# computablee/heterogeneous-spmv

Measured on AMD Instinct MI355X. Metric: SpMV GFLOP/s and achieved HBM GB/s (fp64) per matrix, 1/2/4/8 MI355X, higher is better.
Workload: dtype f64

## Files before the change

### heterogeneous-spmv_amd/cli/cli_common.h

```cpp
#pragma once
#include <math.h>
#include <stdio.h>
#include <stdlib.h>
#include <string.h>

#include <chrono>
#include <string>
#include <vector>

#include "hspmv.h"

namespace cli {

struct Options {
  int gpus = 1;
  int dtype = HSPMV_F64;
  bool x_rand = false;
  unsigned long long seed = 42;
  unsigned kernel = HSPMV_KERNEL_AUTO;
  unsigned lanes = 0;
  bool nt = false;
  int plan = HSPMV_CSR3_PLAN_AUTO;
  int deterministic = 0;
  bool check = true;
  std::string dump_y;
  std::string params = "mi355x";
  bool bandk = true;
};

inline bool ends_with(const std::string &s, const char *suf) {
  const size_t n = strlen(suf);
  return s.size() >= n && s.compare(s.size() - n, n, suf) == 0;
}

inline bool parse_options(int argc, char **argv, int first, Options &o) {
  for (int i = first; i < argc; ++i) {
    std::string a = argv[i];
    auto need = [&](const char *name) -> const char * {
// ... 28 lines not shown
      } else { fprintf(stderr, "bad --kernel %s\n", v); return false; }
    } else if (a == "--nt") {
      o.nt = true;
    } else if (a == "--plan") {
      const char *v = need("--plan"); if (!v) return false;
      if (!strcmp(v, "aligned")) o.plan = HSPMV_CSR3_PLAN_ALIGNED;
      else if (!strcmp(v, "packed")) o.plan = HSPMV_CSR3_PLAN_PACKED;
      else if (!strcmp(v, "ssr")) o.plan = HSPMV_CSR3_PLAN_SSR;
      else { fprintf(stderr, "bad --plan %s\n", v); return false; }
    } else if (a == "--deterministic") {
      o.deterministic = HSPMV_DETERMINISTIC_ORDERED;
    } else if (a == "--reproducible") {
      o.deterministic = HSPMV_DETERMINISTIC_REPRODUCIBLE;
    } else if (a == "--serial") {
      o.deterministic = HSPMV_DETERMINISTIC_SERIAL;
    } else if (a == "--no-check") {
      o.check = false;
    } else if (a == "--dump-y") {
      const char *v = need("--dump-y"); if (!v) return false;
      o.dump_y = v;
    } else if (a == "--file-order") {
      o.bandk = false;
    } else if (a == "--params") {
      const char *v = need("--params"); if (!v) return false;
      o.params = v;
    } else {
      fprintf(stderr, "unknown option %s\n", a.c_str());
      return false;
    }
  }
// ... 64 lines not shown
  int ndev = 0;
  if (hspmv_device_count(&ndev) != HSPMV_OK) return die("hspmv_device_count");
  const int gpus = o.gpus > 0 ? o.gpus : ndev;
  std::vector<int> devs((size_t)(gpus > 0 ? gpus : 1));
  for (size_t p = 0; p < devs.size(); ++p) devs[p] = (int)p;
  hspmv_options opt;
  memset(&opt, 0, sizeof(opt));
  opt.struct_size = sizeof(opt);
  opt.flags = flags_of(o);
  opt.devices = gpus > 1 ? devs.data() : nullptr;
  opt.n_devices = gpus > 1 ? gpus : 0;
  opt.csr3_plan = o.plan;
  opt.deterministic = o.deterministic;
  if (hspmv_create_ex(&h, &view, mv.n_ssr > 0 ? &mv : nullptr, &opt) != HSPMV_OK)
    return die("hspmv_create_ex");
  std::vector<double> x64;
  fill_x(o, A.n, x64);
  if (perm) {
    std::vector<double> xf(x64);
    for (int64_t i = 0; i < A.n; ++i) x64[(size_t)i] = xf[(size_t)perm[i]];
  }
  std::vector<float> x32;
  const void *xp = x64.data();
  if (A.dtype == HSPMV_F32) {
    x32.assign(x64.begin(), x64.end());
    xp = x32.data();
  }
  if (hspmv_set_x(h, xp) != HSPMV_OK) return die("hspmv_set_x");
  hspmv_timing t;
  if (hspmv_run(h, 5, num_runs, &t) != HSPMV_OK) return die("hspmv_run");
// ... 66 lines not shown
```

### heterogeneous-spmv_amd/cli/spmv_csr.cpp

```cpp
#include "cli_common.h"

int main(int argc, char **argv) {
  if (argc < 3) {
    printf("%s inputfile.csr num_runs [--gpus N] [--dtype f32|f64] [--x ones|rand:SEED] "
           "[--kernel auto|stream|vector[:L]] [--nt] [--dump-y PATH] [--no-check]\n",
           argv[0]);
    return 0;
  }
  cli::Options o;
  if (!cli::parse_options(argc, argv, 3, o)) return 1;
  const int num_runs = atoi(argv[2]);
  if (num_runs < 1) {
    fprintf(stderr, "num_runs must be >= 1\n");
    return 1;
  }
  printf("Before Read\n");
  hspmv_csr_buf A;
  hspmv_csr3_buf maps;
  if (cli::read_matrix(argv[1], o.dtype, A, maps) != HSPMV_OK) return cli::die("read");
  printf("After Read\n");
  if (A.dtype != o.dtype) {
    fprintf(stderr, "matrix file holds dtype %d, requested %d\n", A.dtype, o.dtype);
    return 1;
  }
// ... 9 lines not shown
```

### heterogeneous-spmv_amd/csrc/hspmv_api.cpp

```cpp
#include <string.h>

#include <algorithm>
#include <chrono>
#include <cstddef>
#include <memory>
#include <vector>

#include "hspmv_runtime.h"

using namespace hspmv;

namespace {

int check_handle(hspmv_handle *h) {
  if (!h || h->shards.empty()) return set_error(HSPMV_E_INVALID, "invalid handle");
  return HSPMV_OK;
}

int create_single(hspmv_handle **hp, const hspmv_csr *A, const hspmv_csr3_maps *maps, int device,
                  void *stream, unsigned flags, const Tuning &tune) {
  ContigScope contig(tune);
  if (int rc0 = check_deterministic(flags, tune)) return rc0;
  const bool devptrs = (flags & HSPMV_FLAG_DEVICE_PTRS) != 0;
  if (!A) return set_error(HSPMV_E_INVALID, "matrix is NULL");
// ... 68 lines not shown
    }
  }
  if ((rc = finish_shard(s, A->dtype, flags, stream))) {
    free_shard(s, h->borrowed);
    return rc;
  }
  if (!devptrs && (rc = place_shard(s, A->n, A->dtype))) {
    free_shard(s, h->borrowed);
    return rc;
  }
  (void)ncclGetVersion(&h->rccl_version);
  *hp = h.release();
  return HSPMV_OK;
}

int check_devices(const int *devices, int n, int *ndev_out) {
  int ndev = 0;
  if (hipGetDeviceCount(&ndev) != hipSuccess || ndev < 1)
    return set_error(HSPMV_E_NODEV, "no HIP device available");
  *ndev_out = ndev;
  for (int p = 0; devices && p < n; ++p)
    if (devices[p] < 0 || devices[p] >= ndev)
      return set_error(HSPMV_E_NODEV, "device %d out of range (have %d)", devices[p], ndev);
  return HSPMV_OK;
}

}

extern "C" {

// ... 130 lines not shown
  if (!h || gpu < 0 || gpu >= (int)h->shards.size()) return nullptr;
  return (void *)h->shards[gpu].x;
}

void *hspmv_y_device(hspmv_handle *h, int gpu) {
  if (!h || gpu < 0 || gpu >= (int)h->shards.size()) return nullptr;
  return h->shards[gpu].y;
}

int hspmv_spmv(hspmv_handle *h) {
  int rc;
  if ((rc = check_handle(h))) return rc;
  if (!h->x_set) return set_error(HSPMV_E_STATE, "x not set (hspmv_set_x / hspmv_bind_x_device)");
  for (auto &s : h->shards) {
    HIP_TRY(hipSetDevice(s.device));
    hipError_t e = launch_spmv(s.A, s.dp, h->dtype, s.plan, s.x, s.y, s.stream);
    if (e != hipSuccess)
      return set_error(HSPMV_E_HIP, "SpMV launch on GPU %d failed: %s", s.device, hipGetErrorString(e));
  }
  return HSPMV_OK;
}

int hspmv_synchronize(hspmv_handle *h) {
  clear_error();
  int rc;
  if ((rc = check_handle(h))) return rc;
  for (auto &s : h->shards) {
    HIP_TRY(hipSetDevice(s.device));
    HIP_TRY(hipStreamSynchronize(s.stream));
  }
  return HSPMV_OK;
}

int hspmv_run(hspmv_handle *h, int warmup, int iters, hspmv_timing *out) {
  clear_error();
  int rc;
  if ((rc = check_handle(h))) return rc;
  if (!out || iters < 1 || warmup < 0) return set_error(HSPMV_E_INVALID, "bad arguments");
  for (int i = 0; i < warmup; ++i) {
    if ((rc = hspmv_spmv(h))) return rc;
    if ((rc = hspmv_synchronize(h))) return rc;
  }
  double tmin = 1e30, tmax = 0, tsum = 0, wmin = 1e30, wmax = 0, wsum = 0;
  for (int i = 0; i < iters; ++i) {
    auto tic = std::chrono::steady_clock::now();
    for (auto &s : h->shards) {
      HIP_TRY(hipSetDevice(s.device));
      HIP_TRY(hipEventRecord(s.ev0, s.stream));
      hipError_t e = launch_spmv(s.A, s.dp, h->dtype, s.plan, s.x, s.y, s.stream);
      if (e != hipSuccess)
        return set_error(HSPMV_E_HIP, "SpMV launch failed: %s", hipGetErrorString(e));
      HIP_TRY(hipEventRecord(s.ev1, s.stream));
    }
    double dev = 0.0;
    for (auto &s : h->shards) {
      HIP_TRY(hipSetDevice(s.device));
      HIP_TRY(hipEventSynchronize(s.ev1));
      float ms = 0.f;
      HIP_TRY(hipEventElapsedTime(&ms, s.ev0, s.ev1));
      dev = std::max(dev, (double)ms * 1e-3);
    }
    const double wall = std::chrono::duration<double>(std::chrono::steady_clock::now() - tic).count();
    tmin = std::min(tmin, dev); tmax = std::max(tmax, dev); tsum += dev;
    wmin = std::min(wmin, wall); wmax = std::max(wmax, wall); wsum += wall;
  }
  memset(out, 0, sizeof(*out));
  out->t_min = tmin; out->t_max = tmax; out->t_avg = tsum / iters;
  out->wall_min = wmin; out->wall_max = wmax; out->wall_avg = wsum / iters;
// ... 92 lines not shown
  out->csr3_plan = s.plan.kernel != kCsr3 ? 0
                   : s.A.n_ssr == 0 ? HSPMV_CSR3_PLAN_ROW_GROUPS
                   : s.tune.csr3_plan == HSPMV_CSR3_PLAN_SSR ? HSPMV_CSR3_PLAN_SSR
                   : csr3_fill(s.tune) ? HSPMV_CSR3_PLAN_ALIGNED : HSPMV_CSR3_PLAN_PACKED;
  out->csort_slot_bytes = s.plan.kernel == kCsort ? (s.dp.cs.slot32 ? 4 : 8) : 0;
  out->csort_row_blocks = s.plan.kernel == kCsort ? s.dp.cs.row_blocks : 0;
  out->rccl_version = h->rccl_version;
  out->slab_kernel_rule = s.heavy_frac < 0 ? 0 : (s.A.slab_stream ? 2 : 1);
  out->heavy_group_frac = s.heavy_frac < 0 ? 0.0 : s.heavy_frac;
  out->lds_pad = s.plan.lds_pad ? 1 : 0;
  out->csort_fixed_point = s.plan.kernel == kCsort && s.dp.cs.fixed ? 1 : 0;
  out->serial_order = 1;
  for (auto &sh : h->shards) out->serial_order &= sh.dp.serial_max == INT32_MAX ? 1 : 0;
  out->row_slices = s.dp.sl_desc ? 1 : 0;
  out->slice_pos_bits = s.dp.sl_desc ? s.dp.sl_pos_bits : 0;
  if (s.plan.kernel == kCsort)
    for (int hh = 0; hh < 4; ++hh) out->csort_part_begin[hh] = s.csort_part_begin[hh];
  for (auto &sh : h->shards)
    if (sh.plan.kernel == kCsort) {
      out->csort_chunks += sh.csort_chunks;
      out->csort_seg_chunks += sh.csort_seg_chunks;
    }
  return HSPMV_OK;
}

extern "C" {

static_assert(sizeof(hspmv_info) >= HSPMV_INFO_SIZE_1_0, "hspmv_info shrank below its 1.0 layout");
static_assert(offsetof(hspmv_info, heavy_group_frac) + sizeof(double) == HSPMV_INFO_SIZE_1_0,
              "HSPMV_INFO_SIZE_1_0 must end at the last 1.0 field");
// ... 55 lines not shown
```

### heterogeneous-spmv_amd/csrc/hspmv_internal.h

```cpp
#pragma once
#include <hip/hip_runtime_api.h>
#include <stdint.h>

#include "hspmv.h"

namespace hspmv {

struct DevCSR {
  int32_t m = 0;
  int64_t n = 0;
  int64_t nnz = 0;
  const int32_t *row_ptr = nullptr;
  const int32_t *col_idx = nullptr;
  const void *val = nullptr;
  int32_t n_ssr = 0, n_sr = 0;
  const int32_t *outer = nullptr;
  const int32_t *inner = nullptr;
  const uint16_t *col16 = nullptr;
  const int32_t *cbase = nullptr;
  const uint64_t *cplanes = nullptr;
  int32_t n_cplanes = 0, cplane_words = 0;
  int32_t c16_mode = 1;
  int32_t col_span_bits = 0;
  bool has_xwin = false, has_xdict = false;
// ... 61 lines not shown

inline int32_t split_threshold(unsigned flags) {
  return (flags & HSPMV_FLAG_NO_SPLIT) ? INT32_MAX : kLongRow;
}

constexpr double kMallResident = 192.0 * 1024 * 1024;
inline double footprint_bytes(int64_t m, int64_t n, int64_t nnz, int dtype) {
  const double sv = dtype == HSPMV_F64 ? 8.0 : 4.0;
  return (double)nnz * (sv + 4.0) + (double)m * (sv + 4.0) + (double)n * sv;
}
inline bool mall_resident(int64_t m, int64_t n, int64_t nnz, int dtype) {
  return footprint_bytes(m, n, nnz, dtype) <= kMallResident;
}
constexpr double kXcdL2Bytes = 4.0 * 1024 * 1024;

inline unsigned flag_kernel(unsigned flags) { return flags & HSPMV_KERNEL_MASK; }
inline int flag_lanes(unsigned flags) { return (int)((flags & HSPMV_LANES_MASK) >> HSPMV_LANES_SHIFT); }
inline int flag_u(unsigned flags) { return (int)((flags >> HSPMV_U_SHIFT) & 0x1Fu); }
inline int32_t flag_xcd_chunk(unsigned flags) {
  const unsigned code = (flags >> HSPMV_XCD_CHUNK_SHIFT) & 0x1Fu;
  return code ? 1 << (code - 1) : 0;
}
inline int32_t flag_groups(unsigned flags) {
  const unsigned code = (flags >> HSPMV_GROUPS_SHIFT) & 0x7u;
  return code ? 1 << (code - 1) : 1;
}

constexpr int kCsortThreads = 1024;
constexpr int kCsortMaxLds = 160 * 1024;
constexpr int kCsortTraceSlots = 4 + 2 * (kCsortThreads / 64);
// ... 59 lines not shown
  const int32_t *slab_col = nullptr;
  const void *slab_val = nullptr;
  DevCsort cs;
};

struct LaunchPlan {
  int kernel = kStream;
  int lanes = 64;
  int waves_per_block = 4;
  int u = 8;
  bool nontemporal = false;
  bool prefetch = false;
  bool y_nt = false;
  int32_t dyn_lds = 0;
  int32_t xcd_chunk = 1;
  int32_t groups = 1;
  int32_t carry = 0;
  bool lds_pad = false;
  bool row_slices = false;
  int64_t blocks = 0;
};

inline int ssr_waves(double rows_per_ssr) {
  const double w = rows_per_ssr / 64.0;
  return w >= 6.0 ? 8 : (w >= 3.0 ? 4 : (w >= 1.5 ? 2 : 1));
}

LaunchPlan plan_launch(const DevCSR &A, int dtype, unsigned flags, double rows_per_ssr,
                       int64_t packed_tasks, const Tuning &t);

hipError_t launch_rows_f32(const DevCSR &A, const DevPlan &dp, const LaunchPlan &p,
                           const float *x, float *y, hipStream_t st);
hipError_t launch_rows_f64(const DevCSR &A, const DevPlan &dp, const LaunchPlan &p,
                           const double *x, double *y, hipStream_t st);

hipError_t launch_csort(const DevCsort &c, int dtype, const void *x, void *y, hipStream_t st);

hipError_t launch_spmv(const DevCSR &A, const DevPlan &dp, int dtype, const LaunchPlan &plan,
                       const void *x, void *y, hipStream_t stream);

}
```

### heterogeneous-spmv_amd/csrc/hspmv_runtime.h

```cpp
#pragma once
#include <hip/hip_runtime_api.h>
#include <rccl/rccl.h>

#include <algorithm>
#include <cstdint>
#include <thread>
#include <vector>

#include "hspmv_common.h"
#include "hspmv_internal.h"

#define HIP_TRY(expr)                                                              \
  do {                                                                             \
    hipError_t _e = (expr);                                                        \
    if (_e != hipSuccess)                                                          \
      return set_error(HSPMV_E_HIP, "%s failed: %s (%s:%d)", #expr,                \
                       hipGetErrorString(_e), __FILE__, __LINE__);                 \
  } while (0)

namespace hspmv {

struct Shard {
  int device = 0;
  hipStream_t stream = nullptr;
// ... 74 lines not shown
  int64_t m = 0, n = 0, nnz = 0;
  int dtype = HSPMV_F64;
  int64_t n_ssr = 0, n_sr = 0;
  unsigned flags = 0;
  bool x_set = false;
  bool borrowed = false;
  int64_t max_rows = 0;
  bool sharded = false;
  int64_t x_entries() const {
    int64_t t = 0;
    for (auto &s : shards) t += s.x_entries;
    return t;
  }
  std::vector<ncclComm_t> comms;
  int rccl_version = 0;
};

namespace hspmv {

template <typename F>
inline void parallel_ranges(int64_t n, int64_t grain, F &&body) {
  const int nt = (int)std::max<int64_t>(1, std::min<int64_t>(16, n / grain));
  if (nt == 1) return (void)body((int64_t)0, n, 0);
  std::vector<std::thread> th;
  for (int t = 0; t < nt; ++t) th.emplace_back([&, t]() { body(n * t / nt, n * (t + 1) / nt, t); });
  for (auto &x : th) x.join();
}

int tuning_from_options(const hspmv_options *o, Tuning *t);
void tuning_from_env(Tuning *t);
// ... 90 lines not shown
```

### heterogeneous-spmv_amd/csrc/spmv_device.cuh

```cuda
#pragma once
#include <hip/hip_runtime.h>

#include "hspmv_internal.h"

namespace hspmv {
namespace dev {

#ifndef HSPMV_DIAG
#define HSPMV_DIAG 0
#endif

constexpr int kTraceWaves = 1 << 17;
constexpr int kTraceSlots = 8;
#if (HSPMV_DIAG & 8)
static __device__ unsigned long long g_trace[kTraceWaves * kTraceSlots];
__device__ __forceinline__ unsigned long long diag_stamp() {
  unsigned long long t;
  asm volatile("s_waitcnt vmcnt(0) lgkmcnt(0)\n\ts_memtime %0\n\ts_waitcnt lgkmcnt(0)"
               : "=s"(t)::"memory");
  return t;
}
#define HSPMV_TRACE(ts, i, v)            \
  do {                                   \
    if ((ts) != nullptr && lane == 0) (ts)[i] = (v); \
// ... 6 lines not shown
#if (HSPMV_DIAG & 512)
#if !(HSPMV_DIAG & 8)
static __device__ unsigned long long g_trace[kTraceWaves * kTraceSlots];
#endif
__device__ __forceinline__ unsigned long long diag_realtime() {
  unsigned long long t;
  asm volatile("s_memrealtime %0\n\ts_waitcnt lgkmcnt(0)" : "=s"(t)::"memory");
  return t;
}
#endif

constexpr int kWave = 64;
#ifndef HSPMV_COOP_GROUPS
#define HSPMV_COOP_GROUPS 1
#endif
constexpr int kNumXcd = 8;

template <bool PAD>
__device__ __forceinline__ int32_t lds_ix(int32_t i) { return PAD ? i + (i >> 5) : i; }
template <int U, bool PAD>
constexpr int wave_lds() {
  return kWave * U + (PAD ? 2 * U : 0);
}

template <bool NT, typename T>
__device__ __forceinline__ T ldg(const T *p) {
  if constexpr (NT)
    return __builtin_nontemporal_load(p);
  else
    return *p;
}
// ... 44 lines not shown
  v += dpp_move<0x118, 0xf>(v);
  return v;
}

template <typename T>
__device__ __forceinline__ T wave_sum_dpp(T v) {
  v += dpp_move<0x111, 0xf>(v);
  v += dpp_move<0x112, 0xf>(v);
  v += dpp_move<0x114, 0xf>(v);
  v += dpp_move<0x118, 0xf>(v);
  v += dpp_move<0x142, 0xa>(v);
  v += dpp_move<0x143, 0xc>(v);
  return lane_value(v, 63);
}

__device__ __forceinline__ uint32_t xcd_chunk_remap(uint32_t b, uint32_t nb, uint32_t s) {
  if (s <= 1) return b;
  const uint32_t span = kNumXcd * s;
  if (b >= (nb / span) * span) return b;
  const uint32_t i = b / kNumXcd, x = b % kNumXcd;
  return (i / s) * span + x * s + (i % s);
}

__device__ __forceinline__ unsigned long long bits_from(int i) {
  return i >= 64 ? 0ull : (~0ull << i);
}

typedef __attribute__((address_space(1))) const char gchar;

template <bool NT, typename T>
__device__ __forceinline__ T ld_off(const gchar *base, uint32_t byte_off) {
  const __attribute__((address_space(1))) T *p =
      (const __attribute__((address_space(1))) T *)(base + byte_off);
  if constexpr (NT)
    return __builtin_nontemporal_load(p);
  else
    return *p;
// ... 298 lines not shown
    }
    T v[kBatch];
#pragma unroll
    for (int j = 0; j < kBatch; ++j)
      v[j] = ld_off<false, T>(xb, (uint32_t)(min(e[j], total - 1) + d[j]) * (uint32_t)sizeof(T));
#pragma unroll
    for (int j = 0; j < kBatch; ++j)
      if (e[j] < total) xs[e[j]] = v[j];
  }
  __syncthreads();
  if constexpr ((HSPMV_DIAG & (64 | 128)) != 0) __builtin_amdgcn_s_setprio(0);
}

template <typename T, bool NT, int U, bool PF, int C16, bool XW, bool XD, int W = 4, bool PAD = false>
__global__ __launch_bounds__(W * 64) void hspmv_csr_stream(
    int32_t m, int32_t long_t, int32_t serial_max, uint32_t xcd_chunk, int32_t groups, int32_t y_nt,
    int32_t carry,
    const int32_t *__restrict__ rp, ColSrc cs, const int2 *__restrict__ xwin, XDict xd,
    const T *__restrict__ val, const T *__restrict__ x, T *__restrict__ y) {
  static_assert(!XD || W == 4, "dictionaries are planned for 256-row blocks");
  __shared__ T lds[W * wave_lds<U, PAD>()];
  __shared__ T xlds[XW ? W * kXWin : 1];
  extern __shared__ __attribute__((aligned(16))) unsigned char xdyn[];
  const int wid = threadIdx.x >> 6;
  const int lane = threadIdx.x & (kWave - 1);
  const int64_t blk = xcd_chunk_remap(blockIdx.x, gridDim.x, xcd_chunk);
  if constexpr (XD) stage_xdict<T, 256>(reinterpret_cast<T *>(xdyn), x, xd, blk, threadIdx.x);
  int64_t g0 = (blk * W + wid) * (int64_t)groups * kWave;
  if (g0 >= m) return;
  const int64_t gend = min<int64_t>(g0 + (int64_t)groups * kWave, m);
  T *my = lds + wid * wave_lds<U, PAD>();
  unsigned long long *ts = nullptr;
#if (HSPMV_DIAG & 8)
  const int64_t wv = blk * W + wid;
  if (wv < kTraceWaves) ts = g_trace + wv * kTraceSlots;
  HSPMV_TRACE(ts, 0, diag_stamp());
  {
    unsigned hw;
    asm volatile("s_getreg_b32 %0, hwreg(HW_REG_HW_ID)" : "=s"(hw));
    HSPMV_TRACE(ts, 6, (unsigned long long)hw);
  }
// ... 18 lines not shown
    int32_t gbase = 0;
    if constexpr (C16 == 2) gbase = (int32_t)sload_i64(cs.cbase, (uint64_t)(g0 / kWave) * 4u);
    wave_rows<T, NT, U, PF, C16, XW, XD, false, PAD>((int32_t)g0, g1, beg, end, long_t, serial_max, cs, val,
                                                     x, y, my,
                                         lane, win, y_nt != 0, carry != 0, gbase, ts);
    ts = nullptr;
    if (g1 >= gend) break;
    g0 = g1;
    beg = nbeg;
    end = nend;
  }
}

template <typename T, bool NT, int U, bool PF, int C16, int W, bool XW, bool XD>
__global__ __launch_bounds__(W * 64) void hspmv_csr3(
    int32_t n_tasks, int32_t long_t, int32_t serial_max, uint32_t xcd_chunk, int32_t y_nt, int32_t carry,
    int32_t align,
    const int32_t *__restrict__ task_start, const int2 *__restrict__ xwin, XDict xd,
    const int32_t *__restrict__ rp, ColSrc cs, const T *__restrict__ val,
    const T *__restrict__ x, T *__restrict__ y) {
  __shared__ T lds[W * wave_lds<U, false>()];
  __shared__ T xlds[XW ? W * kXWin : 1];
  extern __shared__ __attribute__((aligned(16))) unsigned char xdyn[];
  const int wid = threadIdx.x >> 6;
  const int lane = threadIdx.x & (kWave - 1);
  const int64_t blk = xcd_chunk_remap(blockIdx.x, gridDim.x, xcd_chunk);
#if (HSPMV_DIAG & 512)
  unsigned long long *bt = blk < kTraceWaves ? g_trace + blk * kTraceSlots : nullptr;
  if (bt && threadIdx.x == 0) {
    bt[0] = diag_realtime();
    bt[6] = __builtin_amdgcn_s_getreg((31 << 11) | 4);
    bt[7] = __builtin_amdgcn_s_getreg((31 << 11) | 20);
  }
#endif
  if constexpr (XD) stage_xdict<T, W * 64>(reinterpret_cast<T *>(xdyn), x, xd, blk, threadIdx.x);
  const int64_t t = blk * W + wid;
  if (t >= n_tasks) return;
#if (HSPMV_DIAG & 8)
  const unsigned long long tb_stamp = diag_stamp();
#endif
  const int64_t tb = sload_i64(task_start, (uint64_t)t * 4u);
// ... 161 lines not shown
#pragma unroll
  for (int i = 0; i < B; ++i) {
    const int g = i / 4, r = i % 4;
    const uint32_t p = (full || k0 + 4 * g + 4 <= w) ? slice_pos<PB>(q.pq, i) : q.ps[r < 3 ? r : 0];
    xv[i] = xs[p];
  }
#pragma unroll
  for (int i = 0; i < B; ++i) {
    const T p = q.v[i] * xv[i];
    acc = (k0 + i < len) ? acc + p : acc;
  }
  return acc;
}

template <typename T, bool NT, int B, int PB>
__global__ __launch_bounds__(256) void hspmv_slices(int32_t n_slices, uint32_t xcd_chunk, int32_t y_nt,
                                                    Slices sl, XDict xd, const T *__restrict__ val,
                                                    const T *__restrict__ x, T *__restrict__ y) {
  static_assert(B % 4 == 0 && B >= 4, "batches hold whole position groups");
  static_assert(PB == 16 || (PB == 12 && B % 8 == 0), "12-bit positions come in groups of 8 slots");
  extern __shared__ __attribute__((aligned(16))) unsigned char xdyn[];
  const int wid = threadIdx.x >> 6;
  const int lane = threadIdx.x & (kWave - 1);
  const int64_t blk = xcd_chunk_remap(blockIdx.x, gridDim.x, xcd_chunk);
  const int64_t t = blk * 4 + wid;
  int32_t off = 0, poff = 0, w = 0, r0 = 0, nr = 0;
  if (t < n_slices) {
    const sl_i4 d = sload_i128(sl.desc, (uint64_t)t * 8u);
    off = d[0];
    r0 = d[1];
    w = d[2] - d[0];
    nr = d[3] - d[1];
    poff = PB == 12 ? sload_i32(sl.ppre, (uint64_t)t * 4u) : off;
  }
  int32_t len = 0;
  if (lane < nr) len = (int32_t)sl.len[r0 + lane];
  stage_xdict<T, 256>(reinterpret_cast<T *>(xdyn), x, xd, blk, threadIdx.x);
  if (nr <= 0) return;
  const T *xs = reinterpret_cast<const T *>(xdyn);
// ... 25 lines not shown
  if (w > wf) slice_load_tail<T, NT, B, PB>(tail, vb, pb, wf, w, lane);
  __builtin_amdgcn_sched_barrier(0);
  if (wf > 0) acc = slice_consume<T, B, PB>(acc, cur, xs, wf - B, w, len, true);
  if (w > wf) acc = slice_consume<T, B, 16>(acc, tail, xs, wf, w, len, false);
  if constexpr ((HSPMV_DIAG & 256) != 0) {
    if (lane < nr && acc == T(12345.678)) y[r0 + lane] = acc;
  } else if (lane < nr) {
    if (y_nt)
      __builtin_nontemporal_store(acc, y + r0 + lane);
    else
      y[r0 + lane] = acc;
  }
}


template <typename T, int PB>
void launch_slices_pb(const DevPlan &dp, const LaunchPlan &p, const T *x, T *y, hipStream_t st) {
  const Slices sl{dp.sl_desc, dp.sl_len, dp.sl_pos, dp.sl_ppre};
  const XDict xd{dp.xd_blk, reinterpret_cast<const int2 *>(dp.xd_runs)};
  const unsigned dyn = (unsigned)dp.xd_lds_bytes + (unsigned)p.dyn_lds;
  const T *val = static_cast<const T *>(dp.sl_val);
  if (p.nontemporal)
    hipLaunchKernelGGL((hspmv_slices<T, true, HSPMV_SLICE_BATCH, PB>), dim3((unsigned)p.blocks), dim3(256), dyn,
                       st, dp.n_slices, (uint32_t)p.xcd_chunk, (int32_t)p.y_nt, sl, xd, val, x, y);
  else
    hipLaunchKernelGGL((hspmv_slices<T, false, HSPMV_SLICE_BATCH, PB>), dim3((unsigned)p.blocks), dim3(256), dyn,
                       st, dp.n_slices, (uint32_t)p.xcd_chunk, (int32_t)p.y_nt, sl, xd, val, x, y);
}

template <typename T>
hipError_t launch_slices(const DevPlan &dp, const LaunchPlan &p, const T *x, T *y, hipStream_t st) {
  if (!dp.xd_blk || !dp.sl_len || !dp.sl_pos || !dp.sl_val || p.waves_per_block != 4 ||
      p.blocks != ((int64_t)dp.n_slices + 3) / 4 ||
      !(dp.sl_pos_bits == 16 || (dp.sl_pos_bits == 12 && dp.sl_ppre)))
    return hipErrorInvalidValue;
  if (dp.sl_pos_bits == 12)
    launch_slices_pb<T, 12>(dp, p, x, y, st);
  else
    launch_slices_pb<T, 16>(dp, p, x, y, st);
  return hipGetLastError();
}

inline ColSrc col_src(const DevCSR &A) {
  return ColSrc{A.col_idx, A.col16, A.cbase, A.cplanes, A.n_cplanes, A.cplane_words};
}

template <typename T, bool NT, int U, bool PF, int C16, bool XD>
void launch_rows_u(const DevCSR &A, const DevPlan &dp, const LaunchPlan &p, const T *x, T *y,
                   hipStream_t st) {
  const T *val = static_cast<const T *>(A.val);
  const ColSrc cs = col_src(A);
  const XDict xd{dp.xd_blk, reinterpret_cast<const int2 *>(dp.xd_runs)};
  const unsigned dyn = XD ? (unsigned)dp.xd_lds_bytes + (unsigned)p.dyn_lds : (unsigned)p.dyn_lds;
  if (p.kernel == kStream) {
    const int2 *xw = reinterpret_cast<const int2 *>(dp.xwin);
#define HSPMV_STREAM(C, XW, XDX, W, PAD)                                                            \
  hipLaunchKernelGGL((hspmv_csr_stream<T, NT, U, PF, C, XW, XDX, W, PAD>), dim3((unsigned)p.blocks), \
                     dim3(W * 64), dyn, st, A.m, dp.long_t, dp.serial_max, (uint32_t)p.xcd_chunk,       \
                     (int32_t)p.groups,                                                               \
                     (int32_t)p.y_nt, p.carry, A.row_ptr, cs, xw, xd, val, x, y)
    if constexpr (XD) {
      HSPMV_STREAM(false, false, true, 4, false);
      return;
    }
    if constexpr (!PF) {
      if (p.lds_pad) {
        if (p.waves_per_block == 1 && xw) HSPMV_STREAM(C16, true, false, 1, true);
        else if (p.waves_per_block == 1) HSPMV_STREAM(C16, false, false, 1, true);
        else if (p.waves_per_block != 4 && xw) HSPMV_STREAM(C16, true, false, 2, true);
        else if (p.waves_per_block != 4) HSPMV_STREAM(C16, false, false, 2, true);
        else if (xw) HSPMV_STREAM(C16, true, false, 4, true);
        else HSPMV_STREAM(C16, false, false, 4, true);
        return;
// ... 1 lines not shown
    }
    if (p.waves_per_block == 1 && xw) HSPMV_STREAM(C16, true, false, 1, false);
    else if (p.waves_per_block == 1) HSPMV_STREAM(C16, false, false, 1, false);
    else if (p.waves_per_block != 4 && xw) HSPMV_STREAM(C16, true, false, 2, false);
    else if (p.waves_per_block != 4) HSPMV_STREAM(C16, false, false, 2, false);
    else if (xw) HSPMV_STREAM(C16, true, false, 4, false);
    else HSPMV_STREAM(C16, false, false, 4, false);
#undef HSPMV_STREAM
    return;
  }
  {
  const int2 *xw = reinterpret_cast<const int2 *>(dp.xwin);
#define HSPMV_CSR3(W, C, XW, X)                                                               \
  hipLaunchKernelGGL((hspmv_csr3<T, NT, U, PF, C, W, XW, X>), dim3((unsigned)p.blocks),      \
                     dim3(W * 64), dyn, st, dp.n_tasks, dp.long_t, dp.serial_max,             \
                     (uint32_t)p.xcd_chunk,                                                   \
                     (int32_t)p.y_nt, p.carry, dp.task_align, dp.task_start, xw, xd, A.row_ptr, cs, \
                     val, x, y)
  if constexpr (XD) {
    if (p.waves_per_block == 8)
      HSPMV_CSR3(8, false, false, true);
    else
      HSPMV_CSR3(4, false, false, true);
    return;
  } else {
    if (xw && p.waves_per_block == 4) {
      HSPMV_CSR3(4, C16, true, false);
      return;
    }
    switch (p.waves_per_block) {
      case 1: HSPMV_CSR3(1, C16, false, false); break;
// ... 57 lines not shown
```

### heterogeneous-spmv_amd/csrc/spmv_kernels.hip

```cpp
#include <hip/hip_runtime.h>

#include <cstdlib>

#include "hspmv_internal.h"

namespace hspmv {
namespace {

constexpr int kWave = 64;

template <bool NT, typename T>
__device__ __forceinline__ T ldg(const T *p) {
  if constexpr (NT)
    return __builtin_nontemporal_load(p);
  else
    return *p;
}

template <typename T>
__device__ __forceinline__ T wave_sum(T v) {
#pragma unroll
  for (int off = 32; off > 0; off >>= 1) v += __shfl_xor(v, off, kWave);
  return v;
}
// ... 204 lines not shown
                       dp.long_row, rp, ci, val, x, y, static_cast<T *>(nullptr));
    e = hipGetLastError();
  } else if (dp.n_long > 0) {
    hipLaunchKernelGGL((hspmv_long_chunks<T, NT>), dim3((unsigned)dp.n_chunks), dim3(256), 0, st,
                       dp.n_chunks, dp.chunk_k, ci, val, x, static_cast<T *>(dp.partials));
    hipLaunchKernelGGL((hspmv_long_reduce<T>), dim3((unsigned)((dp.n_long + 3) / 4)), dim3(256),
                       0, st, dp.n_long, dp.long_row, dp.long_cstart,
                       static_cast<const T *>(dp.partials), y);
    e = hipGetLastError();
  }
  return e;
}

}

hipError_t launch_spmv(const DevCSR &A, const DevPlan &dp, int dtype, const LaunchPlan &plan,
                       const void *x, void *y, hipStream_t stream) {
  if (dtype == 1) {
    return plan.nontemporal
               ? launch_typed<double, true>(A, dp, plan, (const double *)x, (double *)y, stream)
               : launch_typed<double, false>(A, dp, plan, (const double *)x, (double *)y, stream);
  }
  return plan.nontemporal
             ? launch_typed<float, true>(A, dp, plan, (const float *)x, (float *)y, stream)
             : launch_typed<float, false>(A, dp, plan, (const float *)x, (float *)y, stream);
}

}
```

### heterogeneous-spmv_amd/hspmv/_lib.py

```python
from __future__ import annotations

import ctypes as C
import os
from pathlib import Path

PKG_ROOT = Path(__file__).resolve().parent.parent
REPO_ROOT = PKG_ROOT.parent
LIB_PATH = Path(os.environ.get("HSPMV_LIB", PKG_ROOT / "build" / "libhspmv.so.1"))
HEADER = REPO_ROOT / "include" / "hspmv.h"

F32, F64 = 0, 1

KERNEL_AUTO, KERNEL_VECTOR, KERNEL_STREAM, KERNEL_CSR3, KERNEL_CSORT = 0, 1, 2, 3, 4
LANES_SHIFT = 4
FLAG_NO_COL16 = 1 << 11
FLAG_NONTEMPORAL = 1 << 12
FLAG_DEVICE_PTRS = 1 << 13
FLAG_NO_XCD_REMAP = 1 << 14
FLAG_NO_SPLIT = 1 << 15
U_SHIFT = 16
FLAG_PREFETCH = 1 << 21
FLAG_XCD_REMAP = 1 << 22
FLAG_COL16 = 1 << 23
XCD_CHUNK_SHIFT = 24
# ... 75 lines not shown
                ("n_split_rows", C.c_int32), ("xcd_remap", C.c_int32), ("groups_per_wave", C.c_int32),
                ("x_entries", C.c_int64), ("format_bytes", C.c_double), ("col16", C.c_int32),
                ("wave_tasks", C.c_int32), ("x_windows", C.c_int32), ("x_dict", C.c_int32),
                ("x_dict_entries", C.c_int64), ("x_slabs", C.c_int32),
                ("col16_group", C.c_int32), ("csort_parts", C.c_int32),
                ("placement_trials", C.c_int32), ("placement_pick", C.c_int32),
                ("placement_us", C.c_double * 8),
                ("deterministic", C.c_int32), ("csr3_plan", C.c_int32),
                ("csort_slot_bytes", C.c_int32), ("csort_row_blocks", C.c_int32),
                ("rccl_version", C.c_int32), ("reserved0", C.c_int32),
                ("csort_chunks", C.c_int64), ("csort_seg_chunks", C.c_int64),
                ("slab_kernel_rule", C.c_int32), ("lds_pad", C.c_int32),
                ("heavy_group_frac", C.c_double),
                ("csort_fixed_point", C.c_int32), ("serial_order", C.c_int32),
                ("csort_part_begin", C.c_int64 * 4),
                ("row_slices", C.c_int32), ("slice_pos_bits", C.c_int32)]


CSR3_PLANS = {"auto": 0, "aligned": 1, "packed": 2, "ssr": 3}
DETERMINISTIC = {"any": 0, "ordered": 1, "reproducible": 2, "serial": 3}
SLICES_WHY = {0: "ok", 1: "off", 2: "no_dict", 3: "shape", 4: "chunked", 5: "split_rows",
              6: "long_row", 7: "bytes", 8: "resident"}
CSR3_PLAN_NAMES = {0: None, 1: "aligned", 2: "packed", 3: "ssr", 4: "row_groups"}


class Options(C.Structure):
    _fields_ = [("struct_size", C.c_uint32), ("flags", C.c_uint32),
                ("devices", C.POINTER(C.c_int)), ("n_devices", C.c_int32),
                ("device", C.c_int32), ("stream", C.c_void_p),
                ("csr3_plan", C.c_int32), ("task_nnz", C.c_int32), ("x_windows", C.c_int32),
                ("x_dict", C.c_int32), ("x_dict_cap", C.c_int32), ("x_slabs", C.c_int32),
                ("col16_group", C.c_int32), ("csort", C.c_int32), ("csort_parts", C.c_int32),
                ("csort_chunk_u", C.c_int32), ("stream_waves", C.c_int32),
                ("deterministic", C.c_int32), ("placement_trials", C.c_int32),
                ("row_slices", C.c_int32)]

    TUNABLE = ("csr3_plan", "task_nnz", "x_windows", "x_dict", "x_dict_cap", "x_slabs",
# ... 29 lines not shown
SIGNATURES = {
    "hspmv_create": (C.c_int, [C.POINTER(_H), C.POINTER(Csr), C.POINTER(Csr3Maps), C.c_int, C.c_uint]),
    "hspmv_create_on_device": (C.c_int, [C.POINTER(_H), C.POINTER(Csr), C.POINTER(Csr3Maps),
                                         C.c_int, _P, C.c_uint]),
    "hspmv_create_sharded": (C.c_int, [C.POINTER(_H), C.POINTER(Csr), C.POINTER(Csr3Maps),
                                       C.POINTER(C.c_int), C.c_int, C.c_uint]),
    "hspmv_create_ex": (C.c_int, [C.POINTER(_H), C.POINTER(Csr), C.POINTER(Csr3Maps),
                                  C.POINTER(Options)]),
    "hspmv_set_x": (C.c_int, [_H, _P]),
    "hspmv_bind_x_device": (C.c_int, [_H, _P]),
    "hspmv_bind_y_device": (C.c_int, [_H, _P]),
    "hspmv_x_device": (_P, [_H, C.c_int]),
    "hspmv_y_device": (_P, [_H, C.c_int]),
    "hspmv_spmv": (C.c_int, [_H]),
    "hspmv_synchronize": (C.c_int, [_H]),
    "hspmv_run": (C.c_int, [_H, C.c_int, C.c_int, C.POINTER(Timing)]),
    "hspmv_get_y": (C.c_int, [_H, _P]),
    "hspmv_exchange": (C.c_int, [_H, C.POINTER(C.c_double), C.POINTER(C.c_double)]),
    "hspmv_get_info": (C.c_int, [_H, C.POINTER(Info)]),
    "hspmv_get_info_sized": (C.c_int, [_H, C.POINTER(Info), C.c_uint32]),
    "hspmv_destroy": (None, [_H]),
    "hspmv_read_csr": (C.c_int, [C.c_char_p, C.c_int, C.POINTER(CsrBuf)]),
    "hspmv_read_mtx": (C.c_int, [C.c_char_p, C.c_int, C.POINTER(CsrBuf)]),
    "hspmv_rcm_reorder": (C.c_int, [C.POINTER(Csr), C.POINTER(CsrBuf), C.c_void_p]),
    "hspmv_read_csr3": (C.c_int, [C.c_char_p, C.c_int, C.POINTER(CsrBuf), C.POINTER(Csr3Buf)]),
    "hspmv_write_csr": (C.c_int, [C.c_char_p, C.POINTER(Csr)]),
    "hspmv_write_csr3": (C.c_int, [C.c_char_p, C.POINTER(Csr), C.POINTER(Csr3Maps)]),
    "hspmv_save_bin": (C.c_int, [C.c_char_p, C.POINTER(Csr), C.POINTER(Csr3Maps)]),
    "hspmv_load_bin": (C.c_int, [C.c_char_p, C.POINTER(CsrBuf), C.POINTER(Csr3Buf)]),
    "hspmv_free_csr": (None, [C.POINTER(CsrBuf)]),
# ... 52 lines not shown
```

### heterogeneous-spmv_amd/hspmv/api.py

```python
from __future__ import annotations

import ctypes as C
from dataclasses import dataclass, field
from typing import Optional

import numpy as np

from . import _lib
from ._lib import (F32, F64, KERNEL_AUTO, KERNEL_CSORT, KERNEL_CSR3, KERNEL_STREAM, KERNEL_VECTOR,
                   FLAG_DEVICE_PTRS, FLAG_NONTEMPORAL, HspmvError, check, lanes_flag, lib,
                   remap_flag)

_KERNELS = {"auto": KERNEL_AUTO, "vector": KERNEL_VECTOR, "stream": KERNEL_STREAM,
            "csr3": KERNEL_CSR3, "csort": KERNEL_CSORT}
KERNEL_NAMES = {v: k for k, v in _KERNELS.items()}


def dtype_code(dtype) -> int:
    dt = np.dtype(dtype)
    if dt == np.float64:
        return F64
    if dt == np.float32:
        return F32
    raise ValueError(f"unsupported dtype {dt} (float32 / float64)")
# ... 379 lines not shown
    def bind_y_device(self, ptr: Optional[int]) -> None:
        check(lib().hspmv_bind_y_device(self._h, ptr), "hspmv_bind_y_device")

    def x_device(self, gpu: int = 0) -> int:
        return lib().hspmv_x_device(self._h, gpu) or 0

    def y_device(self, gpu: int = 0) -> int:
        return lib().hspmv_y_device(self._h, gpu) or 0

    def spmv(self) -> None:
        check(lib().hspmv_spmv(self._h), "hspmv_spmv")

    def synchronize(self) -> None:
        check(lib().hspmv_synchronize(self._h), "hspmv_synchronize")

    def run(self, warmup: int = 5, iters: int = 20) -> dict:
        t = _lib.Timing()
        check(lib().hspmv_run(self._h, int(warmup), int(iters), C.byref(t)), "hspmv_run")
        return {k: getattr(t, k) for k, _ in _lib.Timing._fields_}

    def get_y(self) -> np.ndarray:
        y = np.empty(self.A.m, dtype=self.dtype)
        check(lib().hspmv_get_y(self._h, _ptr(y)), "hspmv_get_y")
        return y

    def __call__(self, x: np.ndarray) -> np.ndarray:
        self.set_x(x)
        self.spmv()
        return self.get_y()

# ... 32 lines not shown
```

### include/hspmv.h

```cpp
#ifndef HSPMV_H
#define HSPMV_H

#include <stdint.h>

#ifdef __cplusplus
extern "C" {
#endif

#define HSPMV_VERSION_MAJOR 1
#define HSPMV_VERSION_MINOR 1

#define HSPMV_OK 0
#define HSPMV_E_INVALID (-1)
#define HSPMV_E_IO (-2)
#define HSPMV_E_NOMEM (-3)
#define HSPMV_E_HIP (-4)
#define HSPMV_E_RCCL (-5)
#define HSPMV_E_NODEV (-6)
#define HSPMV_E_STATE (-7)

typedef enum { HSPMV_F32 = 0, HSPMV_F64 = 1 } hspmv_dtype;

typedef struct {
  int64_t m, n, nnz;
// ... 63 lines not shown
  int32_t csr3_plan;
  int32_t csort_slot_bytes;
  int32_t csort_row_blocks;
  int32_t rccl_version;
  int32_t reserved0;
  int64_t csort_chunks;
  int64_t csort_seg_chunks;
  int32_t slab_kernel_rule;
  int32_t lds_pad;
  double heavy_group_frac;
  int32_t csort_fixed_point;
  int32_t serial_order;
  int64_t csort_part_begin[4];
  int32_t row_slices;
  int32_t slice_pos_bits;
} hspmv_info;

typedef struct hspmv_handle hspmv_handle;

#define HSPMV_KERNEL_AUTO 0u
#define HSPMV_KERNEL_VECTOR 1u
#define HSPMV_KERNEL_STREAM 2u
#define HSPMV_KERNEL_CSR3 3u
#define HSPMV_KERNEL_CSORT 4u
#define HSPMV_KERNEL_MASK 0xFu
#define HSPMV_LANES_SHIFT 4
#define HSPMV_LANES(l) ((unsigned)(l) << HSPMV_LANES_SHIFT)
#define HSPMV_LANES_MASK (0x7Fu << HSPMV_LANES_SHIFT)
#define HSPMV_FLAG_NO_COL16 (1u << 11)
#define HSPMV_FLAG_NONTEMPORAL (1u << 12)
// ... 51 lines not shown
                         const hspmv_csr3_maps *maps, const int *devices,
                         int n_shards, unsigned flags);

int hspmv_create_on_device(hspmv_handle **h, const hspmv_csr *A,
                           const hspmv_csr3_maps *maps, int device,
                           void *stream, unsigned flags);

int hspmv_set_x(hspmv_handle *h, const void *x_host);
int hspmv_bind_x_device(hspmv_handle *h, const void *x_dev);
int hspmv_bind_y_device(hspmv_handle *h, void *y_dev);
void *hspmv_x_device(hspmv_handle *h, int gpu);
void *hspmv_y_device(hspmv_handle *h, int gpu);

int hspmv_spmv(hspmv_handle *h);
int hspmv_synchronize(hspmv_handle *h);

int hspmv_run(hspmv_handle *h, int warmup, int iters, hspmv_timing *out);

int hspmv_get_y(hspmv_handle *h, void *y_host);

int hspmv_exchange(hspmv_handle *h, double *bcast_x_s, double *gather_y_s);

#define HSPMV_INFO_SIZE_1_0 248
int hspmv_get_info(hspmv_handle *h, hspmv_info *out);
int hspmv_get_info_sized(hspmv_handle *h, hspmv_info *out, uint32_t out_size);
void hspmv_destroy(hspmv_handle *h);

int hspmv_read_csr(const char *path, int dtype, hspmv_csr_buf *out);
int hspmv_read_csr3(const char *path, int dtype, hspmv_csr_buf *A,
                    hspmv_csr3_buf *maps);
// ... 55 lines not shown
```

Measured before the change: 1155.

## Alternate block sweep direction between consecutive SpMV launches for cache reuse

Result: faster. 1213 (median of 6 runs) (+5.0%).

```diff
diff --git a/heterogeneous-spmv_amd/cli/cli_common.h b/heterogeneous-spmv_amd/cli/cli_common.h
--- a/heterogeneous-spmv_amd/cli/cli_common.h
+++ b/heterogeneous-spmv_amd/cli/cli_common.h
@@ -22,6 +22,7 @@
   bool nt = false;
   int plan = HSPMV_CSR3_PLAN_AUTO;
   int deterministic = 0;
+  int sweep = HSPMV_SWEEP_AUTO;
   bool check = true;
   std::string dump_y;
   std::string params = "mi355x";
@@ -80,6 +81,11 @@
       o.deterministic = HSPMV_DETERMINISTIC_REPRODUCIBLE;
     } else if (a == "--serial") {
       o.deterministic = HSPMV_DETERMINISTIC_SERIAL;
+    } else if (a == "--sweep") {
+      const char *v = need("--sweep"); if (!v) return false;
+      if (!strcmp(v, "forward")) o.sweep = HSPMV_SWEEP_FORWARD;
+      else if (!strcmp(v, "alternate")) o.sweep = HSPMV_SWEEP_ALTERNATE;
+      else { fprintf(stderr, "bad --sweep %s\n", v); return false; }
     } else if (a == "--no-check") {
       o.check = false;
     } else if (a == "--dump-y") {
@@ -174,6 +180,7 @@
   opt.deterministic = o.deterministic;
   if (hspmv_create_ex(&h, &view, mv.n_ssr > 0 ? &mv : nullptr, &opt) != HSPMV_OK)
     return die("hspmv_create_ex");
+  if (o.sweep != HSPMV_SWEEP_AUTO && hspmv_set_sweep(h, o.sweep) != HSPMV_OK) return die("hspmv_set_sweep");
   std::vector<double> x64;
   fill_x(o, A.n, x64);
   if (perm) {
diff --git a/heterogeneous-spmv_amd/cli/spmv_csr.cpp b/heterogeneous-spmv_amd/cli/spmv_csr.cpp
--- a/heterogeneous-spmv_amd/cli/spmv_csr.cpp
+++ b/heterogeneous-spmv_amd/cli/spmv_csr.cpp
@@ -3,7 +3,8 @@
 int main(int argc, char **argv) {
   if (argc < 3) {
     printf("%s inputfile.csr num_runs [--gpus N] [--dtype f32|f64] [--x ones|rand:SEED] "
-           "[--kernel auto|stream|vector[:L]] [--nt] [--dump-y PATH] [--no-check]\n",
+           "[--kernel auto|stream|vector[:L]] [--nt] [--sweep forward|alternate] [--dump-y PATH] "
+           "[--no-check]\n",
            argv[0]);
     return 0;
   }
diff --git a/heterogeneous-spmv_amd/csrc/hspmv_api.cpp b/heterogeneous-spmv_amd/csrc/hspmv_api.cpp
--- a/heterogeneous-spmv_amd/csrc/hspmv_api.cpp
+++ b/heterogeneous-spmv_amd/csrc/hspmv_api.cpp
@@ -106,6 +106,17 @@
   return HSPMV_OK;
 }
 
+bool shard_alternates(const hspmv_handle *h, const Shard &s) {
+  if (h->sweep_mode == HSPMV_SWEEP_FORWARD || s.A.m == 0) return false;
+  if (s.plan.kernel != kStream && s.plan.kernel != kCsr3) return false;
+  if (h->sweep_mode == HSPMV_SWEEP_ALTERNATE) return true;
+  return s.dp.n_slabs == 0 && !mall_resident(s.A.m, h->n, s.A.nnz, h->dtype);
+}
+
+bool shard_reverse(const hspmv_handle *h, const Shard &s) {
+  return h->sweep_phase && shard_alternates(h, s);
+}
+
 int check_devices(const int *devices, int n, int *ndev_out) {
   int ndev = 0;
   if (hipGetDeviceCount(&ndev) != hipSuccess || ndev < 1)
@@ -266,10 +277,32 @@
   if (!h->x_set) return set_error(HSPMV_E_STATE, "x not set (hspmv_set_x / hspmv_bind_x_device)");
   for (auto &s : h->shards) {
     HIP_TRY(hipSetDevice(s.device));
-    hipError_t e = launch_spmv(s.A, s.dp, h->dtype, s.plan, s.x, s.y, s.stream);
+    hipError_t e = launch_spmv(s.A, s.dp, h->dtype, s.plan, s.x, s.y, s.stream, shard_reverse(h, s));
     if (e != hipSuccess)
       return set_error(HSPMV_E_HIP, "SpMV launch on GPU %d failed: %s", s.device, hipGetErrorString(e));
   }
+  h->sweep_phase = !h->sweep_phase;
+  return HSPMV_OK;
+}
+
+int hspmv_set_sweep(hspmv_handle *h, int mode) {
+  clear_error();
+  int rc;
+  if ((rc = check_handle(h))) return rc;
+  if (mode != HSPMV_SWEEP_AUTO && mode != HSPMV_SWEEP_FORWARD && mode != HSPMV_SWEEP_ALTERNATE)
+    return set_error(HSPMV_E_INVALID, "sweep mode %d (HSPMV_SWEEP_AUTO, _FORWARD or _ALTERNATE)", mode);
+  h->sweep_mode = mode;
+  return HSPMV_OK;
+}
+
+int hspmv_block_order(int64_t n_blocks, int32_t xcd_chunk, int reverse, int32_t *order) {
+  clear_error();
+  if (n_blocks < 0 || n_blocks > INT32_MAX || xcd_chunk < 0 || (n_blocks > 0 && !order))
+    return set_error(HSPMV_E_INVALID, "bad block-order arguments");
+  const uint32_t chunk = (int64_t)xcd_chunk * kNumXcd > n_blocks ? 1u : (uint32_t)xcd_chunk;
+  const uint32_t arg = chunk | (reverse ? kSweepReverse : 0u);
+  for (int64_t b = 0; b < n_blocks; ++b)
+    order[b] = (int32_t)sweep_block((uint32_t)b, (uint32_t)n_blocks, arg);
   return HSPMV_OK;
 }
 
@@ -299,11 +332,12 @@
     for (auto &s : h->shards) {
       HIP_TRY(hipSetDevice(s.device));
       HIP_TRY(hipEventRecord(s.ev0, s.stream));
-      hipError_t e = launch_spmv(s.A, s.dp, h->dtype, s.plan, s.x, s.y, s.stream);
+      hipError_t e = launch_spmv(s.A, s.dp, h->dtype, s.plan, s.x, s.y, s.stream, shard_reverse(h, s));
       if (e != hipSuccess)
         return set_error(HSPMV_E_HIP, "SpMV launch failed: %s", hipGetErrorString(e));
       HIP_TRY(hipEventRecord(s.ev1, s.stream));
     }
+    h->sweep_phase = !h->sweep_phase;
     double dev = 0.0;
     for (auto &s : h->shards) {
       HIP_TRY(hipSetDevice(s.device));
@@ -426,6 +460,7 @@
   for (auto &sh : h->shards) out->serial_order &= sh.dp.serial_max == INT32_MAX ? 1 : 0;
   out->row_slices = s.dp.sl_desc ? 1 : 0;
   out->slice_pos_bits = s.dp.sl_desc ? s.dp.sl_pos_bits : 0;
+  out->sweep = shard_alternates(h, s) ? 1 : 0;
   if (s.plan.kernel == kCsort)
     for (int hh = 0; hh < 4; ++hh) out->csort_part_begin[hh] = s.csort_part_begin[hh];
   for (auto &sh : h->shards)
diff --git a/heterogeneous-spmv_amd/csrc/hspmv_internal.h b/heterogeneous-spmv_amd/csrc/hspmv_internal.h
--- a/heterogeneous-spmv_amd/csrc/hspmv_internal.h
+++ b/heterogeneous-spmv_amd/csrc/hspmv_internal.h
@@ -99,6 +99,27 @@
 }
 constexpr double kXcdL2Bytes = 4.0 * 1024 * 1024;
 
+#if defined(__HIPCC__)
+#define HSPMV_HD __host__ __device__ __forceinline__
+#else
+#define HSPMV_HD inline
+#endif
+constexpr uint32_t kNumXcd = 8;
+
+HSPMV_HD uint32_t xcd_chunk_remap(uint32_t b, uint32_t nb, uint32_t s) {
+  if (s <= 1) return b;
+  const uint32_t span = kNumXcd * s;
+  if (b >= (nb / span) * span) return b;
+  const uint32_t i = b / kNumXcd, x = b % kNumXcd;
+  return (i / s) * span + x * s + (i % s);
+}
+
+constexpr uint32_t kSweepReverse = 0x80000000u;
+HSPMV_HD uint32_t sweep_block(uint32_t b, uint32_t nb, uint32_t order) {
+  const uint32_t blk = xcd_chunk_remap(b, nb, order & ~kSweepReverse);
+  return (order & kSweepReverse) ? nb - 1u - blk : blk;
+}
+
 inline unsigned flag_kernel(unsigned flags) { return flags & HSPMV_KERNEL_MASK; }
 inline int flag_lanes(unsigned flags) { return (int)((flags & HSPMV_LANES_MASK) >> HSPMV_LANES_SHIFT); }
 inline int flag_u(unsigned flags) { return (int)((flags >> HSPMV_U_SHIFT) & 0x1Fu); }
@@ -188,6 +209,7 @@
   bool y_nt = false;
   int32_t dyn_lds = 0;
   int32_t xcd_chunk = 1;
+  bool reverse = false;
   int32_t groups = 1;
   int32_t carry = 0;
   bool lds_pad = false;
@@ -211,6 +233,6 @@
 hipError_t launch_csort(const DevCsort &c, int dtype, const void *x, void *y, hipStream_t st);
 
 hipError_t launch_spmv(const DevCSR &A, const DevPlan &dp, int dtype, const LaunchPlan &plan,
-                       const void *x, void *y, hipStream_t stream);
-
-}
+                       const void *x, void *y, hipStream_t stream, bool reverse = false);
+
+}
diff --git a/heterogeneous-spmv_amd/csrc/hspmv_runtime.h b/heterogeneous-spmv_amd/csrc/hspmv_runtime.h
--- a/heterogeneous-spmv_amd/csrc/hspmv_runtime.h
+++ b/heterogeneous-spmv_amd/csrc/hspmv_runtime.h
@@ -112,6 +112,8 @@
   }
   std::vector<ncclComm_t> comms;
   int rccl_version = 0;
+  int sweep_mode = HSPMV_SWEEP_AUTO;
+  bool sweep_phase = false;
 };
 
 namespace hspmv {
diff --git a/heterogeneous-spmv_amd/csrc/spmv_device.cuh b/heterogeneous-spmv_amd/csrc/spmv_device.cuh
--- a/heterogeneous-spmv_amd/csrc/spmv_device.cuh
+++ b/heterogeneous-spmv_amd/csrc/spmv_device.cuh
@@ -44,7 +44,6 @@
 #ifndef HSPMV_COOP_GROUPS
 #define HSPMV_COOP_GROUPS 1
 #endif
-constexpr int kNumXcd = 8;
 
 template <bool PAD>
 __device__ __forceinline__ int32_t lds_ix(int32_t i) { return PAD ? i + (i >> 5) : i; }
@@ -119,13 +118,6 @@
   return lane_value(v, 63);
 }
 
-__device__ __forceinline__ uint32_t xcd_chunk_remap(uint32_t b, uint32_t nb, uint32_t s) {
-  if (s <= 1) return b;
-  const uint32_t span = kNumXcd * s;
-  if (b >= (nb / span) * span) return b;
-  const uint32_t i = b / kNumXcd, x = b % kNumXcd;
-  return (i / s) * span + x * s + (i % s);
-}
 
 __device__ __forceinline__ unsigned long long bits_from(int i) {
   return i >= 64 ? 0ull : (~0ull << i);
@@ -454,7 +446,7 @@
 
 template <typename T, bool NT, int U, bool PF, int C16, bool XW, bool XD, int W = 4, bool PAD = false>
 __global__ __launch_bounds__(W * 64) void hspmv_csr_stream(
-    int32_t m, int32_t long_t, int32_t serial_max, uint32_t xcd_chunk, int32_t groups, int32_t y_nt,
+    int32_t m, int32_t long_t, int32_t serial_max, uint32_t blk_order, int32_t groups, int32_t y_nt,
     int32_t carry,
     const int32_t *__restrict__ rp, ColSrc cs, const int2 *__restrict__ xwin, XDict xd,
     const T *__restrict__ val, const T *__restrict__ x, T *__restrict__ y) {
@@ -464,7 +456,7 @@
   extern __shared__ __attribute__((aligned(16))) unsigned char xdyn[];
   const int wid = threadIdx.x >> 6;
   const int lane = threadIdx.x & (kWave - 1);
-  const int64_t blk = xcd_chunk_remap(blockIdx.x, gridDim.x, xcd_chunk);
+  const int64_t blk = sweep_block(blockIdx.x, gridDim.x, blk_order);
   if constexpr (XD) stage_xdict<T, 256>(reinterpret_cast<T *>(xdyn), x, xd, blk, threadIdx.x);
   int64_t g0 = (blk * W + wid) * (int64_t)groups * kWave;
   if (g0 >= m) return;
@@ -513,7 +505,7 @@
 
 template <typename T, bool NT, int U, bool PF, int C16, int W, bool XW, bool XD>
 __global__ __launch_bounds__(W * 64) void hspmv_csr3(
-    int32_t n_tasks, int32_t long_t, int32_t serial_max, uint32_t xcd_chunk, int32_t y_nt, int32_t carry,
+    int32_t n_tasks, int32_t long_t, int32_t serial_max, uint32_t blk_order, int32_t y_nt, int32_t carry,
     int32_t align,
     const int32_t *__restrict__ task_start, const int2 *__restrict__ xwin, XDict xd,
     const int32_t *__restrict__ rp, ColSrc cs, const T *__restrict__ val,
@@ -523,7 +515,7 @@
   extern __shared__ __attribute__((aligned(16))) unsigned char xdyn[];
   const int wid = threadIdx.x >> 6;
   const int lane = threadIdx.x & (kWave - 1);
-  const int64_t blk = xcd_chunk_remap(blockIdx.x, gridDim.x, xcd_chunk);
+  const int64_t blk = sweep_block(blockIdx.x, gridDim.x, blk_order);
 #if (HSPMV_DIAG & 512)
   unsigned long long *bt = blk < kTraceWaves ? g_trace + blk * kTraceSlots : nullptr;
   if (bt && threadIdx.x == 0) {
@@ -715,7 +707,7 @@
 }
 
 template <typename T, bool NT, int B, int PB>
-__global__ __launch_bounds__(256) void hspmv_slices(int32_t n_slices, uint32_t xcd_chunk, int32_t y_nt,
+__global__ __launch_bounds__(256) void hspmv_slices(int32_t n_slices, uint32_t blk_order, int32_t y_nt,
                                                     Slices sl, XDict xd, const T *__restrict__ val,
                                                     const T *__restrict__ x, T *__restrict__ y) {
   static_assert(B % 4 == 0 && B >= 4, "batches hold whole position groups");
@@ -723,7 +715,7 @@
   extern __shared__ __attribute__((aligned(16))) unsigned char xdyn[];
   const int wid = threadIdx.x >> 6;
   const int lane = threadIdx.x & (kWave - 1);
-  const int64_t blk = xcd_chunk_remap(blockIdx.x, gridDim.x, xcd_chunk);
+  const int64_t blk = sweep_block(blockIdx.x, gridDim.x, blk_order);
   const int64_t t = blk * 4 + wid;
   int32_t off = 0, poff = 0, w = 0, r0 = 0, nr = 0;
   if (t < n_slices) {
@@ -779,6 +771,10 @@
 }
 
 
+inline uint32_t block_order(const LaunchPlan &p) {
+  return (uint32_t)p.xcd_chunk | (p.reverse ? kSweepReverse : 0u);
+}
+
 template <typename T, int PB>
 void launch_slices_pb(const DevPlan &dp, const LaunchPlan &p, const T *x, T *y, hipStream_t st) {
   const Slices sl{dp.sl_desc, dp.sl_len, dp.sl_pos, dp.sl_ppre};
@@ -787,10 +783,10 @@
   const T *val = static_cast<const T *>(dp.sl_val);
   if (p.nontemporal)
     hipLaunchKernelGGL((hspmv_slices<T, true, HSPMV_SLICE_BATCH, PB>), dim3((unsigned)p.blocks), dim3(256), dyn,
-                       st, dp.n_slices, (uint32_t)p.xcd_chunk, (int32_t)p.y_nt, sl, xd, val, x, y);
+                       st, dp.n_slices, block_order(p), (int32_t)p.y_nt, sl, xd, val, x, y);
   else
     hipLaunchKernelGGL((hspmv_slices<T, false, HSPMV_SLICE_BATCH, PB>), dim3((unsigned)p.blocks), dim3(256), dyn,
-                       st, dp.n_slices, (uint32_t)p.xcd_chunk, (int32_t)p.y_nt, sl, xd, val, x, y);
+                       st, dp.n_slices, block_order(p), (int32_t)p.y_nt, sl, xd, val, x, y);
 }
 
 template <typename T>
@@ -821,7 +817,7 @@
     const int2 *xw = reinterpret_cast<const int2 *>(dp.xwin);
 #define HSPMV_STREAM(C, XW, XDX, W, PAD)                                                            \
   hipLaunchKernelGGL((hspmv_csr_stream<T, NT, U, PF, C, XW, XDX, W, PAD>), dim3((unsigned)p.blocks), \
-                     dim3(W * 64), dyn, st, A.m, dp.long_t, dp.serial_max, (uint32_t)p.xcd_chunk,       \
+                     dim3(W * 64), dyn, st, A.m, dp.long_t, dp.serial_max, block_order(p),       \
                      (int32_t)p.groups,                                                               \
                      (int32_t)p.y_nt, p.carry, A.row_ptr, cs, xw, xd, val, x, y)
     if constexpr (XD) {
@@ -853,7 +849,7 @@
 #define HSPMV_CSR3(W, C, XW, X)                                                               \
   hipLaunchKernelGGL((hspmv_csr3<T, NT, U, PF, C, W, XW, X>), dim3((unsigned)p.blocks),      \
                      dim3(W * 64), dyn, st, dp.n_tasks, dp.long_t, dp.serial_max,             \
-                     (uint32_t)p.xcd_chunk,                                                   \
+                     block_order(p),                                                   \
                      (int32_t)p.y_nt, p.carry, dp.task_align, dp.task_start, xw, xd, A.row_ptr, cs, \
                      val, x, y)
   if constexpr (XD) {
diff --git a/heterogeneous-spmv_amd/csrc/spmv_kernels.hip b/heterogeneous-spmv_amd/csrc/spmv_kernels.hip
--- a/heterogeneous-spmv_amd/csrc/spmv_kernels.hip
+++ b/heterogeneous-spmv_amd/csrc/spmv_kernels.hip
@@ -242,8 +242,10 @@
 
 }
 
-hipError_t launch_spmv(const DevCSR &A, const DevPlan &dp, int dtype, const LaunchPlan &plan,
-                       const void *x, void *y, hipStream_t stream) {
+hipError_t launch_spmv(const DevCSR &A, const DevPlan &dp, int dtype, const LaunchPlan &fwd,
+                       const void *x, void *y, hipStream_t stream, bool reverse) {
+  LaunchPlan plan = fwd;
+  plan.reverse = reverse && (fwd.kernel == kStream || fwd.kernel == kCsr3);
   if (dtype == 1) {
     return plan.nontemporal
                ? launch_typed<double, true>(A, dp, plan, (const double *)x, (double *)y, stream)
diff --git a/heterogeneous-spmv_amd/hspmv/_lib.py b/heterogeneous-spmv_amd/hspmv/_lib.py
--- a/heterogeneous-spmv_amd/hspmv/_lib.py
+++ b/heterogeneous-spmv_amd/hspmv/_lib.py
@@ -113,13 +113,15 @@
                 ("heavy_group_frac", C.c_double),
                 ("csort_fixed_point", C.c_int32), ("serial_order", C.c_int32),
                 ("csort_part_begin", C.c_int64 * 4),
-                ("row_slices", C.c_int32), ("slice_pos_bits", C.c_int32)]
+                ("row_slices", C.c_int32), ("slice_pos_bits", C.c_int32),
+                ("sweep", C.c_int32), ("reserved1", C.c_int32)]
 
 
 CSR3_PLANS = {"auto": 0, "aligned": 1, "packed": 2, "ssr": 3}
 DETERMINISTIC = {"any": 0, "ordered": 1, "reproducible": 2, "serial": 3}
 SLICES_WHY = {0: "ok", 1: "off", 2: "no_dict", 3: "shape", 4: "chunked", 5: "split_rows",
               6: "long_row", 7: "bytes", 8: "resident"}
+SWEEP = {"auto": 0, "forward": 1, "alternate": 2}
 CSR3_PLAN_NAMES = {0: None, 1: "aligned", 2: "packed", 3: "ssr", 4: "row_groups"}
 
 
@@ -179,6 +181,8 @@
     "hspmv_y_device": (_P, [_H, C.c_int]),
     "hspmv_spmv": (C.c_int, [_H]),
     "hspmv_synchronize": (C.c_int, [_H]),
+    "hspmv_set_sweep": (C.c_int, [_H, C.c_int]),
+    "hspmv_block_order": (C.c_int, [C.c_int64, C.c_int32, C.c_int, _P]),
     "hspmv_run": (C.c_int, [_H, C.c_int, C.c_int, C.POINTER(Timing)]),
     "hspmv_get_y": (C.c_int, [_H, _P]),
     "hspmv_exchange": (C.c_int, [_H, C.POINTER(C.c_double), C.POINTER(C.c_double)]),
diff --git a/heterogeneous-spmv_amd/hspmv/api.py b/heterogeneous-spmv_amd/hspmv/api.py
--- a/heterogeneous-spmv_amd/hspmv/api.py
+++ b/heterogeneous-spmv_amd/hspmv/api.py
@@ -417,6 +417,11 @@
     def synchronize(self) -> None:
         check(lib().hspmv_synchronize(self._h), "hspmv_synchronize")
 
+    def set_sweep(self, mode: str) -> None:
+        if mode not in _lib.SWEEP:
+            raise ValueError(f"sweep mode {mode!r} (one of {', '.join(_lib.SWEEP)})")
+        check(lib().hspmv_set_sweep(self._h, _lib.SWEEP[mode]), "hspmv_set_sweep")
+
     def run(self, warmup: int = 5, iters: int = 20) -> dict:
         t = _lib.Timing()
         check(lib().hspmv_run(self._h, int(warmup), int(iters), C.byref(t)), "hspmv_run")
diff --git a/include/hspmv.h b/include/hspmv.h
--- a/include/hspmv.h
+++ b/include/hspmv.h
@@ -101,6 +101,8 @@
   int64_t csort_part_begin[4];
   int32_t row_slices;
   int32_t slice_pos_bits;
+  int32_t sweep;
+  int32_t reserved1;
 } hspmv_info;
 
 typedef struct hspmv_handle hspmv_handle;
@@ -182,6 +184,12 @@
 
 int hspmv_spmv(hspmv_handle *h);
 int hspmv_synchronize(hspmv_handle *h);
+
+#define HSPMV_SWEEP_AUTO 0
+#define HSPMV_SWEEP_FORWARD 1
+#define HSPMV_SWEEP_ALTERNATE 2
+int hspmv_set_sweep(hspmv_handle *h, int mode);
+int hspmv_block_order(int64_t n_blocks, int32_t xcd_chunk, int reverse, int32_t *order);
 
 int hspmv_run(hspmv_handle *h, int warmup, int iters, hspmv_timing *out);
 
```
